# optozorax/portal

Measured on NVIDIA B200. Metric: Mpixels/s @ 3840x2160 depth-40 portal_in_portal, higher is better.
Workload: dtype f32

## Files before the change

portal_b200/csrc/device/pe_glsl.cuh:

```cuda
#pragma once

namespace pe {

#define PE_FI __forceinline__

PE_FI float radians(float d) { return d * 0.017453292519943295f; }
PE_FI float degrees(float r) { return r * 57.29577951308232f; }

PE_FI void pe_sincos_core(float x, float& s, float& c, int& q) {
    float k = ::rintf(x * 0.636619772367581343f);
    float r = ::fmaf(k, -1.5707962513f, x);
    r = ::fmaf(k, -7.5497894159e-08f, r);
    r = ::fmaf(k, -5.3903029535e-15f, r);
    float z = r * r;
    float ps = -1.9515295891e-4f;
    ps = ::fmaf(ps, z, 8.3321608736e-3f);
    ps = ::fmaf(ps, z, -1.6666654611e-1f);
    s = ::fmaf(ps * z, r, r);
    float pc = 2.443315711809948e-5f;
    pc = ::fmaf(pc, z, -1.388731625493765e-3f);
    pc = ::fmaf(pc, z, 4.166664568298827e-2f);
    c = ::fmaf(pc * z, z, ::fmaf(z, -0.5f, 1.0f));
    q = (::fabsf(k) < 1073741824.0f) ? (__float2int_rz(k) & 3) : 0;
}
// ... 116 lines not shown
}
PE_FI float log(float x) { return log2(x) * 0.69314718055994530942f; }
PE_FI float pow(float x, float y) {
    if (y == 0.0f) return 1.0f;
    if (x < 0.0f && y == ::rintf(y)) {
        const float h = y * 0.5f;
        const float r = exp2(y * log2(-x));
        return h != ::rintf(h) ? -r : r;
    }
    return exp2(y * log2(x));
}
PE_FI float sqrt(float x) { return ::sqrtf(x); }
PE_FI float inversesqrt(float x) { return 1.0f / ::sqrtf(x); }
PE_FI float abs(float x) { return ::fabsf(x); }
PE_FI int abs(int x) { return x < 0 ? -x : x; }
PE_FI float sign(float x) { return x > 0.0f ? 1.0f : (x < 0.0f ? -1.0f : 0.0f); }
PE_FI float floor(float x) { return ::floorf(x); }
PE_FI float ceil(float x) { return ::ceilf(x); }
PE_FI float fract(float x) { return x - ::floorf(x); }
PE_FI float mod(float x, float y) { return x - y * ::floorf(x / y); }
PE_FI float min(float x, float y) { return y < x ? y : x; }
PE_FI float max(float x, float y) { return x < y ? y : x; }
PE_FI int min(int x, int y) { return y < x ? y : x; }
PE_FI int max(int x, int y) { return x < y ? y : x; }
PE_FI float clamp(float x, float lo, float hi) { return min(max(x, lo), hi); }
PE_FI int clamp(int x, int lo, int hi) { return min(max(x, lo), hi); }
PE_FI float mix(float x, float y, float a) { return ::fmaf(y, a, x * (1.0f - a)); }
PE_FI float step(float edge, float x) { return x < edge ? 0.0f : 1.0f; }
PE_FI float smoothstep(float e0, float e1, float x) {
    float t = clamp((x - e0) / (e1 - e0), 0.0f, 1.0f);
    return t * t * (3.0f - 2.0f * t);
}

struct vec2;
struct vec3;
struct vec4;

struct swz2_ref {
    float &a, &b;
    PE_FI swz2_ref& operator=(const vec2& v);
    PE_FI swz2_ref& operator+=(const vec2& v);
    PE_FI swz2_ref& operator-=(const vec2& v);
    PE_FI swz2_ref& operator*=(const vec2& v);
    PE_FI swz2_ref& operator/=(const vec2& v);
    PE_FI swz2_ref& operator*=(float s) { a = a * s; b = b * s; return *this; }
    PE_FI swz2_ref& operator/=(float s) { float r = 1.0f / s; a = a * r; b = b * r; return *this; }
    PE_FI swz2_ref& operator+=(float s) { a = a + s; b = b + s; return *this; }
    PE_FI swz2_ref& operator-=(float s) { a = a - s; b = b - s; return *this; }
};
struct swz3_ref {
    float &a, &b, &c;
    PE_FI swz3_ref& operator=(const vec3& v);
    PE_FI swz3_ref& operator+=(const vec3& v);
    PE_FI swz3_ref& operator-=(const vec3& v);
    PE_FI swz3_ref& operator*=(const vec3& v);
    PE_FI swz3_ref& operator/=(const vec3& v);
    PE_FI swz3_ref& operator*=(float s) { a = a * s; b = b * s; c = c * s; return *this; }
    PE_FI swz3_ref& operator/=(float s) { float r = 1.0f / s; a = a * r; b = b * r; c = c * r; return *this; }
    PE_FI swz3_ref& operator+=(float s) { a = a + s; b = b + s; c = c + s; return *this; }
    PE_FI swz3_ref& operator-=(float s) { a = a - s; b = b - s; c = c - s; return *this; }
};
struct swz4_ref {
    float &a, &b, &c, &d;
    PE_FI swz4_ref& operator=(const vec4& v);
    PE_FI swz4_ref& operator+=(const vec4& v);
    PE_FI swz4_ref& operator-=(const vec4& v);
// ... 52 lines not shown
    PE_FI vec4(const vec3& v, float d) : x(v.x), y(v.y), z(v.z), w(d) {}
    PE_FI vec4(float a_, const vec3& v) : x(a_), y(v.x), z(v.y), w(v.z) {}
    PE_FI vec4(const vec2& u, const vec2& v) : x(u.x), y(u.y), z(v.x), w(v.y) {}
    PE_FI vec4(const vec2& u, float c, float d) : x(u.x), y(u.y), z(c), w(d) {}
    PE_FI float& operator[](int i) { return i == 0 ? x : (i == 1 ? y : (i == 2 ? z : w)); }
    PE_FI float operator[](int i) const { return i == 0 ? x : (i == 1 ? y : (i == 2 ? z : w)); }
    PE_SWZ_VEC4
};
#ifndef PE_SWZ_DEFS
#define PE_SWZ_DEFS
#endif
PE_SWZ_DEFS
#define PE_SWZ_ASSIGN(R, V, OPEQ, BODY) PE_FI R& R::operator OPEQ(const V& v) { BODY return *this; }
PE_SWZ_ASSIGN(swz2_ref, vec2, =, a = v.x; b = v.y;)
PE_SWZ_ASSIGN(swz2_ref, vec2, +=, a = a + v.x; b = b + v.y;)
PE_SWZ_ASSIGN(swz2_ref, vec2, -=, a = a - v.x; b = b - v.y;)
PE_SWZ_ASSIGN(swz2_ref, vec2, *=, a = a * v.x; b = b * v.y;)
PE_SWZ_ASSIGN(swz2_ref, vec2, /=, a = a / v.x; b = b / v.y;)
PE_SWZ_ASSIGN(swz3_ref, vec3, =, a = v.x; b = v.y; c = v.z;)
PE_SWZ_ASSIGN(swz3_ref, vec3, +=, a = a + v.x; b = b + v.y; c = c + v.z;)
PE_SWZ_ASSIGN(swz3_ref, vec3, -=, a = a - v.x; b = b - v.y; c = c - v.z;)
PE_SWZ_ASSIGN(swz3_ref, vec3, *=, a = a * v.x; b = b * v.y; c = c * v.z;)
PE_SWZ_ASSIGN(swz3_ref, vec3, /=, a = a / v.x; b = b / v.y; c = c / v.z;)
PE_SWZ_ASSIGN(swz4_ref, vec4, =, a = v.x; b = v.y; c = v.z; d = v.w;)
PE_SWZ_ASSIGN(swz4_ref, vec4, +=, a = a + v.x; b = b + v.y; c = c + v.z; d = d + v.w;)
PE_SWZ_ASSIGN(swz4_ref, vec4, -=, a = a - v.x; b = b - v.y; c = c - v.z; d = d - v.w;)
PE_SWZ_ASSIGN(swz4_ref, vec4, *=, a = a * v.x; b = b * v.y; c = c * v.z; d = d * v.w;)
PE_SWZ_ASSIGN(swz4_ref, vec4, /=, a = a / v.x; b = b / v.y; c = c / v.z; d = d / v.w;)
#undef PE_SWZ_ASSIGN
PE_FI vec2::vec2(const vec3& v) : x(v.x), y(v.y) {}
PE_FI vec2::vec2(const vec4& v) : x(v.x), y(v.y) {}
PE_FI vec3::vec3(const vec4& v) : x(v.x), y(v.y), z(v.z) {}

#define PE_V2(EX, EY) vec2(EX, EY)
#define PE_V3(EX, EY, EZ) vec3(EX, EY, EZ)
#define PE_V4(EX, EY, EZ, EW) vec4(EX, EY, EZ, EW)
#define PE_BINOPS(OP)                                                                                              \
    PE_FI vec2 operator OP(const vec2& a, const vec2& b) { return PE_V2(a.x OP b.x, a.y OP b.y); }                 \
    PE_FI vec2 operator OP(const vec2& a, float s) { return PE_V2(a.x OP s, a.y OP s); }                           \
    PE_FI vec2 operator OP(float s, const vec2& a) { return PE_V2(s OP a.x, s OP a.y); }                           \
    PE_FI vec3 operator OP(const vec3& a, const vec3& b) { return PE_V3(a.x OP b.x, a.y OP b.y, a.z OP b.z); }     \
    PE_FI vec3 operator OP(const vec3& a, float s) { return PE_V3(a.x OP s, a.y OP s, a.z OP s); }                 \
    PE_FI vec3 operator OP(float s, const vec3& a) { return PE_V3(s OP a.x, s OP a.y, s OP a.z); }                 \
    PE_FI vec4 operator OP(const vec4& a, const vec4& b) {                                                         \
        return PE_V4(a.x OP b.x, a.y OP b.y, a.z OP b.z, a.w OP b.w);                                              \
    }                                                                                                              \
    PE_FI vec4 operator OP(const vec4& a, float s) { return PE_V4(a.x OP s, a.y OP s, a.z OP s, a.w OP s); }       \
    PE_FI vec4 operator OP(float s, const vec4& a) { return PE_V4(s OP a.x, s OP a.y, s OP a.z, s OP a.w); }
PE_BINOPS(+)
PE_BINOPS(-)
PE_BINOPS(*)
#undef PE_BINOPS
PE_FI vec2 operator/(const vec2& a, const vec2& b) { return vec2(a.x / b.x, a.y / b.y); }
PE_FI vec3 operator/(const vec3& a, const vec3& b) { return vec3(a.x / b.x, a.y / b.y, a.z / b.z); }
PE_FI vec4 operator/(const vec4& a, const vec4& b) { return vec4(a.x / b.x, a.y / b.y, a.z / b.z, a.w / b.w); }
PE_FI vec2 operator/(float s, const vec2& a) { return vec2(s / a.x, s / a.y); }
PE_FI vec3 operator/(float s, const vec3& a) { return vec3(s / a.x, s / a.y, s / a.z); }
PE_FI vec4 operator/(float s, const vec4& a) { return vec4(s / a.x, s / a.y, s / a.z, s / a.w); }
PE_FI vec2 operator/(const vec2& a, float s) { float r = 1.0f / s; return vec2(a.x * r, a.y * r); }
PE_FI vec3 operator/(const vec3& a, float s) { float r = 1.0f / s; return vec3(a.x * r, a.y * r, a.z * r); }
PE_FI vec4 operator/(const vec4& a, float s) { float r = 1.0f / s; return vec4(a.x * r, a.y * r, a.z * r, a.w * r); }
PE_FI vec2 operator-(const vec2& a) { return vec2(-a.x, -a.y); }
PE_FI vec3 operator-(const vec3& a) { return vec3(-a.x, -a.y, -a.z); }
PE_FI vec4 operator-(const vec4& a) { return vec4(-a.x, -a.y, -a.z, -a.w); }

#define PE_COMPOUND(V)                                                      \
    PE_FI V& operator+=(V& a, const V& b) { a = a + b; return a; }          \
    PE_FI V& operator-=(V& a, const V& b) { a = a - b; return a; }          \
    PE_FI V& operator*=(V& a, const V& b) { a = a * b; return a; }          \
    PE_FI V& operator/=(V& a, const V& b) { a = a / b; return a; }          \
    PE_FI V& operator+=(V& a, float s) { a = a + s; return a; }             \
    PE_FI V& operator-=(V& a, float s) { a = a - s; return a; }             \
    PE_FI V& operator*=(V& a, float s) { a = a * s; return a; }             \
    PE_FI V& operator/=(V& a, float s) { a = a / s; return a; }
PE_COMPOUND(vec2)
PE_COMPOUND(vec3)
PE_COMPOUND(vec4)
#undef PE_COMPOUND

PE_FI bool operator==(const vec2& a, const vec2& b) { return a.x == b.x && a.y == b.y; }
PE_FI bool operator==(const vec3& a, const vec3& b) { return a.x == b.x && a.y == b.y && a.z == b.z; }
PE_FI bool operator==(const vec4& a, const vec4& b) { return a.x == b.x && a.y == b.y && a.z == b.z && a.w == b.w; }
PE_FI bool operator!=(const vec2& a, const vec2& b) { return !(a == b); }
// ... 361 lines not shown
```

portal_b200/csrc/pe_api.cpp:

```cpp
#include <cuda_runtime.h>
#include <dlfcn.h>
#include <nvrtc.h>
#include <sys/stat.h>
#include <unistd.h>

#include <cmath>
#include <cstdio>
#include <cstdlib>
#include <cstring>
#include <fstream>
#include <map>
#include <memory>
#include <mutex>
#include <string>
#include <type_traits>
#include <vector>

#include "../../include/portal_b200.h"
#include "pe_codegen.h"
#include "pe_driver.h"
#include "pe_internal.h"
#include "pe_kernels.h"

using namespace pe_host;

namespace {

struct PeLaunchHost {
    void* out;
    void* bounces;
    int32_t width, height;
    int32_t strip_rows, strip_first, strip_step, n_strips;
    int32_t out_full_frame;
    int32_t tiles_x, tiles_y;
    int32_t out_rgba8;
    void* queue;
    int32_t strip_shift;
    int32_t pad_;
};
static_assert(sizeof(PeLaunchHost) == 72, "PeLaunch layout");

struct Variant {
    std::string source;
    std::vector<char> cubin;
    CUmodule_t module = nullptr;
    CUfunction_t kernel = nullptr;
    CUfunction_t probe = nullptr;
    CUdeviceptr_t const_ptr = 0;
    size_t const_size = 0;
    int regs = 0;
    int blocks_per_sm = 1;
    CUmodule_t module2 = nullptr;
    CUfunction_t kernel2 = nullptr;
    CUdeviceptr_t const_ptr2 = 0;
};

struct Texture {
    void* dev = nullptr;
    int w = 0, h = 0;
};

std::string g_create_error;
std::mutex g_create_mutex;

uint64_t fnv1a(const std::string& s, uint64_t h) {
    for (unsigned char c : s) {
        h ^= c;
        h *= 1099511628211ull;
    }
    return h;
}

std::string lib_dir() {
    Dl_info info;
    if (dladdr((void*)&fnv1a, &info) && info.dli_fname) {
        std::string p = info.dli_fname;
        size_t s = p.rfind('/');
        return s == std::string::npos ? "." : p.substr(0, s);
    }
    return ".";
}

std::string cache_dir() {
    const char* e = std::getenv("PORTAL_B200_CACHE_DIR");
    std::string d = e && *e ? e : lib_dir() + "/_cache";
    mkdir(d.c_str(), 0755);
    return d;
// ... 184 lines not shown
            const float v = m[16 * slot + e];
            if (!std::isfinite(v)) finite = false;
            if (v == 0.0f) z |= 1u << e;
            else if (v == 1.0f) o |= 1u << e;
        }
        if (bottom_row_only) {
            const bool affine = (z & 0x0888u) == 0x0888u && (o & 0x8000u);
            z = affine ? 0x0888u : 0u;
            o = affine ? 0x8000u : 0u;
            if (!affine) finite = false;
        }
        return std::pair<unsigned, unsigned>{z, o | (finite ? 1u << 16 : 0u)};
    };
    for (int k = 0; k < c->layout.n_mat; k++) out[size_t(k)] = masks_of(k, false);
    const int cams[3] = {c->layout.camera_slot, c->layout.camera_slot + 2, c->layout.camera_slot + 3};
    for (int q = 0; q < 3; q++) out[size_t(c->layout.n_mat + q)] = masks_of(cams[q], true);
    return out;
}

std::vector<int> variant_key(pe_ctx* c, const std::vector<int>& ints, const std::vector<std::pair<unsigned, unsigned>>& masks) {
    std::vector<int> key;
    if (c->opts.specialize_ints) {
        key = ints;
        key[c->layout.int_slot["_ray_tracing_depth"]] = 0;
        key[c->layout.int_slot["_aa_start"]] = 0;
    }
    if (c->opts.specialize_matrices)
        for (auto& zo : masks) { key.push_back(int(zo.first)); key.push_back(int(zo.second)); }
    key.push_back(c->opts.with_probe ? 1 : 0);
    key.push_back(c->opts.uniforms_in_smem);
    key.push_back(c->opts.tile_w);
    key.push_back(c->opts.canon_rays ? 1 : 0);
    key.push_back(c->opts.w_aware ? 1 : 0);
    key.push_back(c->opts.block_threads);
    key.push_back(c->opts.min_blocks);
    key.push_back(c->opts.persistent ? 1 : 0);
    for (char d : c->opts.dynamic_ints) key.push_back(d);
    for (char d : c->opts.dynamic_mats) key.push_back(d);
    return key;
}

struct NvrtcApi {
    nvrtcResult (*Version)(int*, int*) = nullptr;
    nvrtcResult (*CreateProgram)(nvrtcProgram*, const char*, const char*, int, const char* const*, const char* const*) = nullptr;
    nvrtcResult (*CompileProgram)(nvrtcProgram, int, const char* const*) = nullptr;
    nvrtcResult (*GetProgramLogSize)(nvrtcProgram, size_t*) = nullptr;
    nvrtcResult (*GetProgramLog)(nvrtcProgram, char*) = nullptr;
    nvrtcResult (*GetCUBINSize)(nvrtcProgram, size_t*) = nullptr;
    nvrtcResult (*GetCUBIN)(nvrtcProgram, char*) = nullptr;
    nvrtcResult (*DestroyProgram)(nvrtcProgram*) = nullptr;
    const char* (*GetErrorString)(nvrtcResult) = nullptr;
    std::string why;
    bool ok = false;
};
const NvrtcApi& nvrtc_api() {
    static NvrtcApi api;
    static std::once_flag once;
    std::call_once(once, [] {
        void* h = nullptr;
        const char* env = std::getenv("PORTAL_B200_NVRTC");
        const char* candidates[] = {env && *env ? env : nullptr,
#ifdef PE_NVRTC_PATH
                                    PE_NVRTC_PATH,
#endif
                                    "/usr/local/cuda/lib64/libnvrtc.so.12", "libnvrtc.so.12", "libnvrtc.so"};
        for (const char* cnd : candidates) {
// ... 85 lines not shown

const int kMaxRespecialisations = 4;

bool select_variant(pe_ctx* c) {
    ensure_layout(c);
    std::vector<int> ints = current_ints(c);
    std::vector<std::pair<unsigned, unsigned>> masks = matrix_masks(c);
    if (c->adapt) {
        c->opts.dynamic_ints.resize(ints.size(), 0);
        c->opts.dynamic_mats.resize(masks.size(), 0);
        c->int_changes.resize(ints.size(), 0);
        c->mat_changes.resize(masks.size(), 0);
        if (c->last_ints.size() == ints.size())
            for (size_t k = 0; k < ints.size(); k++)
                if (ints[k] != c->last_ints[k] && ++c->int_changes[k] > kMaxRespecialisations) c->opts.dynamic_ints[k] = 1;
        if (c->last_masks.size() == masks.size())
            for (size_t k = 0; k < masks.size(); k++)
                if (masks[k] != c->last_masks[k] && ++c->mat_changes[k] > kMaxRespecialisations) c->opts.dynamic_mats[k] = 1;
        c->last_ints = ints;
        c->last_masks = masks;
    }
    for (size_t k = 0; k < ints.size() && k < c->opts.dynamic_ints.size(); k++)
        if (c->opts.dynamic_ints[k]) ints[k] = 0;
    for (size_t k = 0; k < masks.size() && k < c->opts.dynamic_mats.size(); k++)
        if (c->opts.dynamic_mats[k]) masks[k] = {0u, 0u};
    std::vector<int> key = variant_key(c, ints, masks);
    auto it = c->variants.find(key);
    if (it == c->variants.end()) {
        if (c->variants.size() >= 64) {
            for (auto v = c->variants.begin(); v != c->variants.end();) {
                if (v->second.get() == c->current) { ++v; continue; }
                if (v->second->module && c->has_gpu) { cudaDeviceSynchronize(); c->drv->cuModuleUnload(v->second->module); }
                if (v->second->module2 && c->has_gpu) c->drv->cuModuleUnload(v->second->module2);
                v = c->variants.erase(v);
            }
        }
        GenResult g = generate_program(c->scene, c->layout, c->opts, ints, masks);
        if (!g.error.empty()) {
            c->err = g.error;
            return false;
        }
        auto v = std::make_unique<Variant>();
        v->source = std::move(g.source);
        if (!compile_cubin(c, v->source, v->cubin)) return false;
        it = c->variants.emplace(key, std::move(v)).first;
    }
    Variant* v = it->second.get();
    if (c->has_gpu && !v->module) {
        const DriverApi* d = c->drv;
        CUresult_t r = d->cuModuleLoadData(&v->module, v->cubin.data());
        if (r != 0) {
            if (!compile_cubin(c, v->source, v->cubin, true)) return false;
            r = d->cuModuleLoadData(&v->module, v->cubin.data());
        }
        if (r != 0) { c->err = "cuModuleLoadData: " + driver_error(d, r); return false; }
        r = d->cuModuleGetFunction(&v->kernel, v->module, "pe_render_kernel");
        if (r != 0) { c->err = "cuModuleGetFunction(pe_render_kernel): " + driver_error(d, r); return false; }
        const char* block_symbol = c->opts.uniforms_in_smem ? "PE_C_UPLOAD" : "PE_C";
        r = d->cuModuleGetGlobal(&v->const_ptr, &v->const_size, v->module, block_symbol);
        if (r != 0) { c->err = std::string("cuModuleGetGlobal(") + block_symbol + "): " + driver_error(d, r); return false; }
        if (v->const_size != c->layout.size) { c->err = "constant block size mismatch between host and device"; return false; }
        if (c->opts.with_probe) {
            r = d->cuModuleGetFunction(&v->probe, v->module, "pe_probe_kernel");
            if (r != 0) { c->err = "cuModuleGetFunction(pe_probe_kernel): " + driver_error(d, r); return false; }
        }
        d->cuFuncGetAttribute(&v->regs, 4 , v->kernel);
// ... 56 lines not shown
        if (e != cudaSuccess) {
            g_create_error = std::string("cudaSetDevice: ") + cudaGetErrorString(e);
            return nullptr;
        }
        cudaDeviceProp prop;
        if (cudaGetDeviceProperties(&prop, device) == cudaSuccess) {
            c->sm_count = prop.multiProcessorCount;
            if (prop.major < 10) {
                g_create_error = "portal_b200 needs an sm_100a (B200) device; found sm_" + std::to_string(prop.major) +
                                 std::to_string(prop.minor);
                return nullptr;
            }
        }
        if (cudaStreamCreateWithFlags(&c->stream, cudaStreamNonBlocking) != cudaSuccess ||
            cudaMalloc(&c->queue_dev, 256) != cudaSuccess) {
            g_create_error = "cannot create stream / queue counter";
            if (c->stream) cudaStreamDestroy(c->stream);
            return nullptr;
        }
        c->has_gpu = true;
    }
    g_create_error.clear();
    return c.release();
}

void pe_destroy(pe_ctx* c) {
    if (!c) return;
    if (c->has_gpu) {
        cudaSetDevice(c->device);
        cudaDeviceSynchronize();
        for (auto& kv : c->variants) {
            if (kv.second->module) c->drv->cuModuleUnload(kv.second->module);
            if (kv.second->module2) c->drv->cuModuleUnload(kv.second->module2);
        }
        for (auto& kv : c->textures)
            if (kv.second.dev) cudaFree(kv.second.dev);
        if (c->scratch_dev) cudaFree(c->scratch_dev);
        if (c->scratch8_dev) cudaFree(c->scratch8_dev);
        for (auto& sl : c->slots) {
            if (sl.dev) cudaFree(sl.dev);
            if (sl.rendered) cudaEventDestroy(sl.rendered);
            if (sl.copied) cudaEventDestroy(sl.copied);
        }
        for (auto& kv : c->user_scratch)
            if (kv.second.dev) cudaFree(kv.second.dev);
        if (c->ustage) cudaFreeHost(c->ustage);
        for (auto& e : c->ustage_done) if (e) cudaEventDestroy(e);
        if (c->copy_stream) cudaStreamDestroy(c->copy_stream);
        if (c->queue_dev) cudaFree(c->queue_dev);
        if (c->stream) cudaStreamDestroy(c->stream);
    }
    delete c;
}

const char* pe_last_error(pe_ctx* c) { return c ? c->err.c_str() : g_create_error.c_str(); }

int pe_scene_begin(pe_ctx* c) {
    if (!c) return 1;
    if (c->has_gpu) {
        cudaSetDevice(c->device);
        cudaDeviceSynchronize();
        for (auto& kv : c->variants) {
            if (kv.second->module) c->drv->cuModuleUnload(kv.second->module);
            if (kv.second->module2) c->drv->cuModuleUnload(kv.second->module2);
        }
    }
    c->variants.clear();
    c->current = nullptr;
    c->scene = SceneDesc();
    c->layout_valid = false;
    c->last_ints.clear();
    c->int_changes.clear();
    c->last_masks.clear();
    c->mat_changes.clear();
    c->opts.dynamic_ints.clear();
    c->opts.dynamic_mats.clear();
    c->cblock.clear();
    c->pending_mat.clear();
    c->pending_f.clear();
    c->pending_i.clear();
    return 0;
}

#define PE_NEED(c, p)                                  \
    if (!(c)) return 1;                                \
    if (!(p)) return (c)->fail("null argument: " #p);  \
    if ((c)->layout_valid) return (c)->fail("scene description is frozen (uniforms were already set or compiled); call pe_scene_begin")

int pe_scene_add_library(pe_ctx* c, const char* name, const char* glsl) {
    PE_NEED(c, name && glsl);
    c->scene.library.push_back({name, glsl});
    return 0;
}

int pe_scene_add_material_simple(pe_ctx* c, const char* name, const double color[3], double normal_coef, int grid,
                                 double grid_scale, double grid_coef, int grid2, int grid3) {
    PE_NEED(c, name && color);
// ... 88 lines not shown
    return 0;
}

int pe_scene_declare_texture(pe_ctx* c, const char* name) {
    PE_NEED(c, name);
    c->scene.textures.push_back(name);
    return 0;
}

int pe_scene_set_skybox(pe_ctx* c, const char* texture_name) {
    PE_NEED(c, texture_name);
    c->scene.skybox = texture_name;
    return 0;
}

int pe_set_option(pe_ctx* c, const char* key, int value) {
    if (!c || !key) return 1;
    std::string k = key;
    if (k == "persistent") c->opts.persistent = value != 0;
    else if (k == "specialize_ints") c->opts.specialize_ints = value != 0;
    else if (k == "block_threads") {
        if (value < 64 || value > 1024 || value % 64) return c->fail("block_threads must be a multiple of 64 in [64, 1024]");
        c->opts.block_threads = value;
    } else if (k == "min_blocks") c->opts.min_blocks = value < 1 ? 1 : value;
    else if (k == "lineinfo") c->lineinfo = value != 0;
    else if (k == "unroll_loops") c->opts.unroll_loops = value != 0;
    else if (k == "specialize_matrices") c->opts.specialize_matrices = value != 0;
    else if (k == "hoist_planes") c->opts.hoist_planes = value != 0;
    else if (k == "lazy_planes") c->opts.lazy_planes = value != 0;
    else if (k == "with_probe") c->opts.with_probe = value != 0;
    else if (k == "adaptive") c->adapt = value != 0;
    else if (k == "canon_rays") c->opts.canon_rays = value != 0;
    else if (k == "w_aware") c->opts.w_aware = value != 0;
    else if (k == "uniforms_in_smem") {
        if (value < 0 || value > 2) return c->fail("uniforms_in_smem must be 0 (constant bank), 1 (copy loop) or 2 (TMA bulk copy)");
        c->opts.uniforms_in_smem = value;
    } else if (k == "tile_w") {
        if (value != 8 && value != 16 && value != 32) return c->fail("tile_w must be 8, 16 or 32");
        c->opts.tile_w = value;
    }
    else return c->fail("unknown option `" + k + "`");
    if (c->has_gpu) {
        cudaSetDevice(c->device);
        cudaDeviceSynchronize();
        for (auto& kv : c->variants) {
            if (kv.second->module) c->drv->cuModuleUnload(kv.second->module);
            if (kv.second->module2) c->drv->cuModuleUnload(kv.second->module2);
        }
    }
    c->variants.clear();
    c->current = nullptr;
    return 0;
}

int pe_scene_compile(pe_ctx* c) {
    if (!c) return 1;
    if (c->opts.block_threads % 64) return c->fail("block_threads must be a multiple of 64");
    return select_variant(c) ? 0 : 1;
}

const char* pe_scene_source(pe_ctx* c) { return (c && c->current) ? c->current->source.c_str() : ""; }

int pe_scene_cubin(pe_ctx* c, const void** data, size_t* size) {
    if (!c || !data || !size) return 1;
    if (!c->current) return c->fail("no compiled program");
    *data = c->current->cubin.data();
    *size = c->current->cubin.size();
    return 0;
}

int pe_scene_uniform_block(pe_ctx* c, int width, int height, const void** data, size_t* size) {
    if (!c || !data || !size) return 1;
    if (width <= 0 || height <= 0) return c->fail("pe_scene_uniform_block: bad frame size");
    ensure_layout(c);
    *fslot(c, c->layout.float_slot["_resolution_x"]) = float(width);
    *fslot(c, c->layout.float_slot["_resolution_y"]) = float(height);
    if (!select_variant(c)) return 1;
    update_derived(c);
    *data = c->cblock.data();
    *size = c->cblock.size();
// ... 74 lines not shown
    return 0;
}

size_t pe_target_pixels(const pe_target* t) {
    if (!t) return 0;
    if (t->full_frame_layout) return size_t(t->width) * size_t(t->height);
    return size_t(t->n_strips) * size_t(t->strip_rows) * size_t(t->width);
}

static bool upload_uniform_block(pe_ctx* c, CUdeviceptr_t dst, CUstream_t s) {
    const size_t n = c->cblock.size();
    const size_t stride = (n + 255) & ~size_t(255);
    if (!c->ustage || c->ustage_stride < stride) {
        if (c->ustage) { cudaDeviceSynchronize(); cudaFreeHost(c->ustage); c->ustage = nullptr; }
        if (!cuda_ok(c, cudaHostAlloc(reinterpret_cast<void**>(&c->ustage), stride * pe_ctx::kStage, cudaHostAllocDefault), "cudaHostAlloc(uniform staging)")) return false;
        c->ustage_stride = stride;
        for (int k = 0; k < pe_ctx::kStage; k++) {
            c->ustage_used[k] = false;
            if (!c->ustage_done[k] && !cuda_ok(c, cudaEventCreateWithFlags(&c->ustage_done[k], cudaEventDisableTiming), "event")) return false;
        }
    }
    const int k = c->ustage_next;
    c->ustage_next = (k + 1) % pe_ctx::kStage;
    if (c->ustage_used[k] && !cuda_ok(c, cudaEventSynchronize(c->ustage_done[k]), "uniform staging")) return false;
    uint8_t* src = c->ustage + size_t(k) * c->ustage_stride;
    std::memcpy(src, c->cblock.data(), n);
    CUresult_t r = c->drv->cuMemcpyHtoDAsync(dst, src, n, s);
    if (r != 0) { c->err = "uniform block upload: " + driver_error(c->drv, r); return false; }
    if (!cuda_ok(c, cudaEventRecord(c->ustage_done[k], (cudaStream_t)s), "event record")) return false;
    c->ustage_used[k] = true;
    return true;
}

static int render_impl(pe_ctx* c, const pe_target* t, void* out_device, void* bounces_device, void* stream, bool rgba8, int instance = 0) {
    if (!c) return 1;
    if (!out_device) return c->fail("pe_render: out_device is null");
    if (!check_target(c, t) || !bind_device(c)) return 1;
    if (t->n_strips == 0) return 0;
    ensure_layout(c);
    *fslot(c, c->layout.float_slot["_resolution_x"]) = float(t->width);
    *fslot(c, c->layout.float_slot["_resolution_y"]) = float(t->height);
    if (!select_variant(c)) return 1;
    update_derived(c);
    Variant* v = c->current;
    const DriverApi* d = c->drv;
    CUstream_t s = stream ? (CUstream_t)stream : (CUstream_t)c->stream;

    CUfunction_t kernel = v->kernel;
    CUdeviceptr_t const_ptr = v->const_ptr;
    CUresult_t r = 0;
    if (instance == 1) {
        if (!v->module2) {
            size_t sz = 0;
            r = d->cuModuleLoadData(&v->module2, v->cubin.data());
            if (r == 0) r = d->cuModuleGetFunction(&v->kernel2, v->module2, "pe_render_kernel");
            if (r == 0) r = d->cuModuleGetGlobal(&v->const_ptr2, &sz, v->module2, c->opts.uniforms_in_smem ? "PE_C_UPLOAD" : "PE_C");
            if (r != 0) return c->fail("second program instance: " + driver_error(d, r));
        }
        kernel = v->kernel2;
        const_ptr = v->const_ptr2;
    }
    if (!upload_uniform_block(c, const_ptr, s)) return 1;

    PeLaunchHost L;
    std::memset(&L, 0, sizeof L);
    L.out = out_device;
    L.bounces = bounces_device;
    L.width = t->width;
    L.height = t->height;
    L.strip_rows = t->strip_rows;
    L.strip_first = t->strip_first;
    L.strip_step = t->strip_step;
    L.n_strips = t->n_strips;
    L.out_full_frame = t->full_frame_layout ? 1 : 0;
    const int local_rows = t->n_strips * t->strip_rows;
    L.tiles_x = (t->width + 7) / 8;
    L.tiles_y = (local_rows + 3) / 4;
    L.out_rgba8 = rgba8 ? 1 : 0;
    L.queue = c->queue_dev;
    L.strip_shift = -1;
    if ((t->strip_rows & (t->strip_rows - 1)) == 0)
        for (int sh = 0; sh < 31; sh++)
            if ((1 << sh) == t->strip_rows) L.strip_shift = sh;
    void* args[] = {&L};
    unsigned gx, gy;
    if (c->opts.persistent) {
        r = d->cuMemsetD32Async((CUdeviceptr_t)c->queue_dev, 0, 1, s);
        if (r != 0) return c->fail("queue reset: " + driver_error(d, r));
        gx = unsigned(c->sm_count * v->blocks_per_sm);
        gy = 1;
    } else {
        const int tile_w = c->opts.tile_w, block_w = tile_w < 16 ? 16 : tile_w;
        const int rows_per_block = (c->opts.block_threads / 32) / (block_w / tile_w) * (32 / tile_w);
        gx = unsigned((t->width + block_w - 1) / block_w);
        gy = unsigned((local_rows + rows_per_block - 1) / rows_per_block);
    }
    r = d->cuLaunchKernel(kernel, gx, gy, 1, unsigned(c->opts.block_threads), 1, 1, 0, s, args, nullptr);
    if (r != 0) return c->fail("cuLaunchKernel(pe_render_kernel): " + driver_error(d, r));
    c->launches++;
    return 0;
}

}
int pe_internal_render_impl(pe_ctx* c, const pe_target* t, void* out_device, void* stream, int rgba8, int instance) {
    return render_impl(c, t, out_device, nullptr, stream, rgba8 != 0, instance);
}
extern "C" {

int pe_render(pe_ctx* c, const pe_target* t, void* out_device, void* bounces_device, void* stream) {
    return render_impl(c, t, out_device, bounces_device, stream, false);
}

int pe_render_rgba8(pe_ctx* c, const pe_target* t, void* out_device_rgba8, void* stream) {
    return render_impl(c, t, out_device_rgba8, nullptr, stream, true);
}

static bool ensure_scratch(pe_ctx* c, void** p, size_t* have, size_t need);

int pe_probe_ray(pe_ctx* c, const float a[3], const float b[3], float pos_out[3], int32_t* have_result,
                 int32_t* encounter_object, int32_t* change_subspace) {
    if (!c) return 1;
    if (!a || !b || !pos_out) return c->fail("pe_probe_ray: null argument");
    if (!bind_device(c)) return 1;
    ensure_layout(c);
    auto tl = c->layout.int_slot.find("teleport_light_u");
    int saved = 0;
    if (tl != c->layout.int_slot.end()) { saved = *islot(c, tl->second); *islot(c, tl->second) = 1; }
    const bool had_probe = c->opts.with_probe, had_adapt = c->adapt;
    c->opts.with_probe = true;
    c->adapt = false;
    bool ok = select_variant(c);
    c->adapt = had_adapt;
    if (ok) update_derived(c);
    struct { float ax, ay, az, bx, by, bz; void* out; } P;
    float host[6] = {0, 0, 0, 0, 0, 0};
    if (ok) {
        if (!ensure_scratch(c, &c->scratch8_dev, &c->scratch8_bytes, 64)) ok = false;
    }
    if (ok) {
        Variant* v = c->current;
        const DriverApi* d = c->drv;
        CUstream_t s = (CUstream_t)c->stream;
        P = {a[0], a[1], a[2], b[0], b[1], b[2], c->scratch8_dev};
        void* args[] = {&P};
        CUresult_t r = upload_uniform_block(c, v->const_ptr, s) ? 0 : 999;
        if (r == 0) r = d->cuLaunchKernel(v->probe, 1, 1, 1, 32, 1, 1, 0, s, args, nullptr);
        if (r != 0) { c->err = "pe_probe_kernel: " + driver_error(d, r); ok = false; }
        else {
            c->launches++;
            ok = cuda_ok(c, cudaMemcpyAsync(host, c->scratch8_dev, sizeof host, cudaMemcpyDeviceToHost, c->stream), "probe readback") &&
                 cuda_ok(c, cudaStreamSynchronize(c->stream), "pe_probe_ray");
        }
    }
    c->opts.with_probe = had_probe;
    if (tl != c->layout.int_slot.end()) *islot(c, tl->second) = saved;
    if (!ok) return 1;
    for (int k = 0; k < 3; k++) pos_out[k] = host[k];
    if (have_result) *have_result = host[3] != 0.0f;
    if (encounter_object) *encounter_object = host[4] != 0.0f;
    if (change_subspace) *change_subspace = host[5] != 0.0f;
    return 0;
}

static bool ensure_scratch(pe_ctx* c, void** p, size_t* have, size_t need) {
    if (*have >= need) return true;
    if (*p) cudaFree(*p);
    *p = nullptr;
    *have = 0;
    if (!cuda_ok(c, cudaMalloc(p, need), "cudaMalloc(staging)")) return false;
    *have = need;
    return true;
}

int pe_render_host(pe_ctx* c, const pe_target* t, float* out_host) {
    if (!c) return 1;
    if (!out_host) return c->fail("pe_render_host: out_host is null");
    if (!check_target(c, t) || !bind_device(c)) return 1;
    size_t bytes = pe_target_pixels(t) * 16;
// ... 328 lines not shown
```

portal_b200/csrc/pe_codegen.cpp:

```cpp
#include "pe_codegen.h"

#include <algorithm>
#include <cctype>
#include <cmath>
#include <cstdio>
#include <cstring>
#include <sstream>
#include <stdexcept>

#include "../../include/portal_b200.h"

namespace pe_host {

const char* const kRendererFloats[] = {"_camera_scale", "_tan_half_view", "_view_angle", "_t_start", "_t_end",
                                       "_offset_after_material", "_depth_map_min", "_depth_map_max",
                                       "_resolution_x", "_resolution_y", "_left_eye_scale", "_right_eye_scale",
                                       "_panini_param", "_anaglyph_p", "_anaglyph_q"};
const int kNumRendererFloats = int(sizeof(kRendererFloats) / sizeof(kRendererFloats[0]));
const char* const kRendererInts[] = {"_ray_tracing_depth", "_aa_start", "_aa_count", "_camera_in_subspace",
                                     "_darken_by_distance", "_angle_color_disable", "_grid_disable",
                                     "_black_border_disable", "_draw_depth_map", "_left_eye_in_subspace",
                                     "_right_eye_in_subspace", "_use_panini_projection", "_use_360_camera",
                                     "_use_180_camera", "_draw_side_by_side", "_draw_anaglyph", "_anaglyph_mode"};
const int kNumRendererInts = int(sizeof(kRendererInts) / sizeof(kRendererInts[0]));
// ... 462 lines not shown
        if (o.matrix_a != o.matrix_b && !need_mat(o.matrix_b + "_to_" + o.matrix_a, "_mat_teleport")) break;
        body.line("    } else if (i.material == teleport_" + std::to_string(pos) + "_1_M) {");
        body.line("        return material_teleport(hit, r, " + ab + ");");
        body.line("    } else if (i.material == teleport_" + std::to_string(pos) + "_2_M) {");
        body.line("        return material_teleport(hit, r, " + ba + ");");
    }
    body.line("    }");
    body.line("    return material_final(vec3(0.0f));");
    body.line("}");

    body.line("PE_FI SceneIntersectionWithMaterial scene_intersect_material_process(const Ray& r) {");
    body.line("    SceneIntersectionWithMaterial result = SceneIntersectionWithMaterial{scene_intersection_none, material_empty()};");
    if (!scene.intersection_materials.empty())
        body.line("    SceneIntersectionWithMaterial hit = result;");
    for (size_t pos = 0; pos < scene.intersection_materials.size(); pos++) {
        body.line("    hit = intersect_material_" + std::to_string(pos) + "(r);");
        body.line("    if (nearer(result.scene.hit, hit.scene.hit)) { result = hit; }");
    }
    body.line("    (void)r; return result;");
    body.line("}");

    if (!body.err.empty() && R.error.empty()) R.error = body.err;
    if (!R.error.empty()) return R;

    std::ostringstream hd;
    hd << "// GENERATED by portal_b200 (pe_codegen.cpp) -- sm_100a program of one scene.\n";
    hd << "#define PE_PERSISTENT " << (opts.persistent ? 1 : 0) << "\n";
    hd << "#define PE_BLOCK_THREADS " << opts.block_threads << "\n";
    hd << "#define PE_MIN_BLOCKS " << opts.min_blocks << "\n";
    hd << "#define PE_WITH_PROBE " << (opts.with_probe ? 1 : 0) << "\n";
    hd << "#define PE_TILE_W " << opts.tile_w << "\n";
    hd << "#define PE_CANON_RAYS " << (opts.canon_rays ? 1 : 0) << "\n";
    hd << "#define PE_W_AWARE " << ((opts.w_aware && opts.canon_rays) ? 1 : 0) << "\n";
    std::string swz_err;
    hd << "#define PE_SWZ_VEC2" << swizzle_macro(body.swz, 2) << lvalue_swizzle_macro(body.swz_w, 2, swz_err) << "\n";
    hd << "#define PE_SWZ_VEC3" << swizzle_macro(body.swz, 3) << lvalue_swizzle_macro(body.swz_w, 3, swz_err) << "\n";
    hd << "#define PE_SWZ_VEC4" << swizzle_macro(body.swz, 4) << lvalue_swizzle_macro(body.swz_w, 4, swz_err) << "\n";
    hd << "#define PE_SWZ_DEFS" << swizzle_macro(body.swz, 0) << "\n";
    if (!swz_err.empty()) { R.error = swz_err; return R; }
    hd << "#define PE_HAS_SKYBOX " << (scene.skybox.empty() ? 0 : 1) << "\n";
    {
        std::string user;
        for (const auto& lib : scene.library) user += lib.code + "\n";
        for (const char* fn : {"transpose", "inverse", "determinant"}) {
            bool defined = false;
            for (const char* ty : {"mat2", "mat3", "mat4", "float"}) {
                size_t pos = 0;
                const std::string needle = std::string(ty);
                while ((pos = user.find(needle, pos)) != std::string::npos) {
                    size_t k = pos + needle.size();
                    size_t k0 = k;
                    while (k < user.size() && std::isspace((unsigned char)user[k])) k++;
                    if (k > k0 && user.compare(k, std::strlen(fn), fn) == 0) {
                        size_t e = k + std::strlen(fn);
                        while (e < user.size() && std::isspace((unsigned char)user[e])) e++;
                        if (e < user.size() && user[e] == '(' && (pos == 0 || !is_ident_char(user[pos - 1]))) defined = true;
                    }
                    pos = k0;
                }
            }
            if (defined) hd << "#define PE_NO_BUILTIN_" << fn << "\n";
        }
    }
    hd << kSrcGlsl << "\n";
    hd << "namespace pe {\n";
    hd << "// Constant uniform block: scene matrices + camera, floats, ints, texture descriptors.\n";
// ... 95 lines not shown
```

portal_b200/csrc/pe_codegen.h:

```cpp
#pragma once
#include <cstdint>
#include <map>
#include <set>
#include <string>
#include <vector>

namespace pe_host {

enum class ObjClass { Flat, Complex, DebugMatrix };
enum class MatType { Simple, Reflect, Refract, Complex };

struct Material {
    std::string name;
    MatType type = MatType::Simple;
    double color[3] = {0, 0, 0};
    double normal_coef = 0, grid_scale = 0, grid_coef = 0, refractive_index = 0;
    bool grid = false, grid2 = false, grid3 = false;
    std::string code;
};

struct Object {
    std::string name;
    ObjClass cls = ObjClass::Flat;
    bool portal = false;
// ... 26 lines not shown
extern const char* const kRendererInts[];
extern const int kNumRendererInts;

struct PlaneRec {
    int mat_slot = 0;
    int pass_sign = 1;
    int cmp_sign = 1;
};

struct ConstLayout {
    int n_mat = 0, n_float = 0, n_int = 0, n_tex = 0;
    std::vector<std::string> mats, floats, ints;
    std::map<std::string, int> mat_slot, float_slot, int_slot, tex_slot;
    size_t off_mat = 0, off_float = 0, off_int = 0, off_tex = 0, size = 0;
    std::vector<PlaneRec> planes;
    int plane_f0 = 0, plane_i0 = 0;
    int camera_slot = 0;
};
ConstLayout make_layout(const SceneDesc& scene);

struct GenOptions {
    bool persistent = false;
    bool specialize_ints = true;
    int block_threads = 512;
    int min_blocks = 2;
    bool specialize_matrices = true;
    bool hoist_planes = true;
    bool lazy_planes = true;
    bool with_probe = false;
    int uniforms_in_smem = 0;
    int tile_w = 8;
    bool canon_rays = true;
    bool w_aware = true;
    bool unroll_loops = true;
    std::vector<char> dynamic_ints, dynamic_mats;
};

struct GenResult {
    std::string source;
    std::string error;
};

GenResult generate_program(const SceneDesc& scene, const ConstLayout& layout, const GenOptions& opts,
                           const std::vector<int>& int_values,
                           const std::vector<std::pair<unsigned, unsigned>>& matrix_masks);

std::string glsl_to_cuda(const std::string& glsl, std::set<std::string>& swizzles, bool keep_loops_rolled = false,
                         std::set<std::string>* lvalue_swizzles = nullptr);

extern const char* const kSrcGlsl;
extern const char* const kSrcLibrary;
extern const char* const kSrcKernel;

}
```

Baseline: 16850.

## Add optional packed f32x2 vector add/sub and skip redundant uniform uploads

Routes vec2/3/4 addition and subtraction through a pe_f2 helper. Behind a new pack_f32x2 option, which is off by default, that helper can use the paired __fadd2_rn instruction. Separately, each variant now keeps a copy of the uniform block resident on the device per instance and skips re-uploading it when nothing has changed. A second-instance render can also reuse instance 0's constant buffer, with an event to order any later upload. The goal is to cut per-frame host-to-device copies and, optionally, the FP32 instruction count, at the cost of added event bookkeeping and a risk of ordering hazards.

```diff
diff --git a/portal_b200/csrc/device/pe_glsl.cuh b/portal_b200/csrc/device/pe_glsl.cuh
--- a/portal_b200/csrc/device/pe_glsl.cuh
+++ b/portal_b200/csrc/device/pe_glsl.cuh
@@ -172,6 +172,21 @@
     return t * t * (3.0f - 2.0f * t);
 }
 
+#ifndef PE_PACK_F32X2
+#define PE_PACK_F32X2 0
+#endif
+struct pe_f2 { float x, y; };
+#if PE_PACK_F32X2 && defined(__CUDA_ARCH__)
+PE_FI float2 pe_to2(pe_f2 a) { return make_float2(a.x, a.y); }
+PE_FI pe_f2 pe_from2(float2 a) { return pe_f2{a.x, a.y}; }
+PE_FI pe_f2 pe_add2(pe_f2 a, pe_f2 b) { return pe_from2(__fadd2_rn(pe_to2(a), pe_to2(b))); }
+PE_FI pe_f2 pe_sub2(pe_f2 a, pe_f2 b) { return pe_from2(__fadd2_rn(pe_to2(a), make_float2(-b.x, -b.y))); }
+#else
+PE_FI pe_f2 pe_add2(pe_f2 a, pe_f2 b) { return pe_f2{a.x + b.x, a.y + b.y}; }
+PE_FI pe_f2 pe_sub2(pe_f2 a, pe_f2 b) { return pe_f2{a.x - b.x, a.y - b.y}; }
+#endif
+PE_FI pe_f2 pe_bc2(float s) { return pe_f2{s, s}; }
+
 struct vec2;
 struct vec3;
 struct vec4;
@@ -290,6 +305,26 @@
 PE_FI vec2::vec2(const vec4& v) : x(v.x), y(v.y) {}
 PE_FI vec3::vec3(const vec4& v) : x(v.x), y(v.y), z(v.z) {}
 
+PE_FI pe_f2 pe_xy(const vec2& v) { return pe_f2{v.x, v.y}; }
+PE_FI pe_f2 pe_xy(const vec3& v) { return pe_f2{v.x, v.y}; }
+PE_FI pe_f2 pe_xy(const vec4& v) { return pe_f2{v.x, v.y}; }
+PE_FI pe_f2 pe_zw(const vec4& v) { return pe_f2{v.z, v.w}; }
+PE_FI vec2 pe_v2(pe_f2 xy) { return vec2(xy.x, xy.y); }
+PE_FI vec3 pe_v3(pe_f2 xy, float z) { return vec3(xy.x, xy.y, z); }
+PE_FI vec4 pe_v4(pe_f2 xy, pe_f2 zw) { return vec4(xy.x, xy.y, zw.x, zw.y); }
+#define PE_BINOPS2(OP, F2)                                                                                                \
+    PE_FI vec2 operator OP(const vec2& a, const vec2& b) { return pe_v2(F2(pe_xy(a), pe_xy(b))); }                        \
+    PE_FI vec2 operator OP(const vec2& a, float s) { return pe_v2(F2(pe_xy(a), pe_bc2(s))); }                             \
+    PE_FI vec2 operator OP(float s, const vec2& a) { return pe_v2(F2(pe_bc2(s), pe_xy(a))); }                             \
+    PE_FI vec3 operator OP(const vec3& a, const vec3& b) { return pe_v3(F2(pe_xy(a), pe_xy(b)), a.z OP b.z); }            \
+    PE_FI vec3 operator OP(const vec3& a, float s) { return pe_v3(F2(pe_xy(a), pe_bc2(s)), a.z OP s); }                   \
+    PE_FI vec3 operator OP(float s, const vec3& a) { return pe_v3(F2(pe_bc2(s), pe_xy(a)), s OP a.z); }                   \
+    PE_FI vec4 operator OP(const vec4& a, const vec4& b) { return pe_v4(F2(pe_xy(a), pe_xy(b)), F2(pe_zw(a), pe_zw(b))); } \
+    PE_FI vec4 operator OP(const vec4& a, float s) { return pe_v4(F2(pe_xy(a), pe_bc2(s)), F2(pe_zw(a), pe_bc2(s))); }     \
+    PE_FI vec4 operator OP(float s, const vec4& a) { return pe_v4(F2(pe_bc2(s), pe_xy(a)), F2(pe_bc2(s), pe_zw(a))); }
+PE_BINOPS2(+, pe_add2)
+PE_BINOPS2(-, pe_sub2)
+#undef PE_BINOPS2
 #define PE_V2(EX, EY) vec2(EX, EY)
 #define PE_V3(EX, EY, EZ) vec3(EX, EY, EZ)
 #define PE_V4(EX, EY, EZ, EW) vec4(EX, EY, EZ, EW)
@@ -305,8 +340,6 @@
     }                                                                                                              \
     PE_FI vec4 operator OP(const vec4& a, float s) { return PE_V4(a.x OP s, a.y OP s, a.z OP s, a.w OP s); }       \
     PE_FI vec4 operator OP(float s, const vec4& a) { return PE_V4(s OP a.x, s OP a.y, s OP a.z, s OP a.w); }
-PE_BINOPS(+)
-PE_BINOPS(-)
 PE_BINOPS(*)
 #undef PE_BINOPS
 PE_FI vec2 operator/(const vec2& a, const vec2& b) { return vec2(a.x / b.x, a.y / b.y); }
diff --git a/portal_b200/csrc/pe_api.cpp b/portal_b200/csrc/pe_api.cpp
--- a/portal_b200/csrc/pe_api.cpp
+++ b/portal_b200/csrc/pe_api.cpp
@@ -53,6 +53,9 @@
     CUmodule_t module2 = nullptr;
     CUfunction_t kernel2 = nullptr;
     CUdeviceptr_t const_ptr2 = 0;
+    std::vector<uint8_t> resident[2];
+    cudaEvent_t borrowed = nullptr;
+    bool borrow_pending = false;
 };
 
 struct Texture {
@@ -303,6 +306,7 @@
     key.push_back(c->opts.tile_w);
     key.push_back(c->opts.canon_rays ? 1 : 0);
     key.push_back(c->opts.w_aware ? 1 : 0);
+    key.push_back(c->opts.pack_f32x2 ? 1 : 0);
     key.push_back(c->opts.block_threads);
     key.push_back(c->opts.min_blocks);
     key.push_back(c->opts.persistent ? 1 : 0);
@@ -454,6 +458,7 @@
                 if (v->second.get() == c->current) { ++v; continue; }
                 if (v->second->module && c->has_gpu) { cudaDeviceSynchronize(); c->drv->cuModuleUnload(v->second->module); }
                 if (v->second->module2 && c->has_gpu) c->drv->cuModuleUnload(v->second->module2);
+                if (v->second->borrowed && c->has_gpu) cudaEventDestroy(v->second->borrowed);
                 v = c->variants.erase(v);
             }
         }
@@ -576,6 +581,7 @@
         for (auto& kv : c->variants) {
             if (kv.second->module) c->drv->cuModuleUnload(kv.second->module);
             if (kv.second->module2) c->drv->cuModuleUnload(kv.second->module2);
+            if (kv.second->borrowed) cudaEventDestroy(kv.second->borrowed);
         }
         for (auto& kv : c->textures)
             if (kv.second.dev) cudaFree(kv.second.dev);
@@ -607,6 +613,7 @@
         for (auto& kv : c->variants) {
             if (kv.second->module) c->drv->cuModuleUnload(kv.second->module);
             if (kv.second->module2) c->drv->cuModuleUnload(kv.second->module2);
+            if (kv.second->borrowed) cudaEventDestroy(kv.second->borrowed);
         }
     }
     c->variants.clear();
@@ -761,6 +768,7 @@
     else if (k == "adaptive") c->adapt = value != 0;
     else if (k == "canon_rays") c->opts.canon_rays = value != 0;
     else if (k == "w_aware") c->opts.w_aware = value != 0;
+    else if (k == "pack_f32x2") c->opts.pack_f32x2 = value != 0;
     else if (k == "uniforms_in_smem") {
         if (value < 0 || value > 2) return c->fail("uniforms_in_smem must be 0 (constant bank), 1 (copy loop) or 2 (TMA bulk copy)");
         c->opts.uniforms_in_smem = value;
@@ -775,6 +783,7 @@
         for (auto& kv : c->variants) {
             if (kv.second->module) c->drv->cuModuleUnload(kv.second->module);
             if (kv.second->module2) c->drv->cuModuleUnload(kv.second->module2);
+            if (kv.second->borrowed) cudaEventDestroy(kv.second->borrowed);
         }
     }
     c->variants.clear();
@@ -915,6 +924,18 @@
     return true;
 }
 
+static bool ensure_uniform_block(pe_ctx* c, Variant* v, int inst, CUstream_t s) {
+    std::vector<uint8_t>& res = v->resident[inst];
+    if (res == c->cblock) return true;
+    if (inst == 0 && v->borrow_pending) {
+        if (!cuda_ok(c, cudaStreamWaitEvent((cudaStream_t)s, v->borrowed, 0), "uniform block ordering")) return false;
+        v->borrow_pending = false;
+    }
+    if (!upload_uniform_block(c, inst == 0 ? v->const_ptr : v->const_ptr2, s)) { res.clear(); return false; }
+    res = c->cblock;
+    return true;
+}
+
 static int render_impl(pe_ctx* c, const pe_target* t, void* out_device, void* bounces_device, void* stream, bool rgba8, int instance = 0) {
     if (!c) return 1;
     if (!out_device) return c->fail("pe_render: out_device is null");
@@ -930,8 +951,12 @@
     CUstream_t s = stream ? (CUstream_t)stream : (CUstream_t)c->stream;
 
     CUfunction_t kernel = v->kernel;
-    CUdeviceptr_t const_ptr = v->const_ptr;
     CUresult_t r = 0;
+    const bool borrow = instance == 1 && v->resident[0] == c->cblock;
+    if (borrow) {
+        if (!v->borrowed && !cuda_ok(c, cudaEventCreateWithFlags(&v->borrowed, cudaEventDisableTiming), "event")) return 1;
+        instance = 0;
+    }
     if (instance == 1) {
         if (!v->module2) {
             size_t sz = 0;
@@ -941,9 +966,8 @@
             if (r != 0) return c->fail("second program instance: " + driver_error(d, r));
         }
         kernel = v->kernel2;
-        const_ptr = v->const_ptr2;
-    }
-    if (!upload_uniform_block(c, const_ptr, s)) return 1;
+    }
+    if (!ensure_uniform_block(c, v, instance, s)) return 1;
 
     PeLaunchHost L;
     std::memset(&L, 0, sizeof L);
@@ -980,6 +1004,10 @@
     }
     r = d->cuLaunchKernel(kernel, gx, gy, 1, unsigned(c->opts.block_threads), 1, 1, 0, s, args, nullptr);
     if (r != 0) return c->fail("cuLaunchKernel(pe_render_kernel): " + driver_error(d, r));
+    if (borrow) {
+        if (!cuda_ok(c, cudaEventRecord(v->borrowed, (cudaStream_t)s), "event record")) return 1;
+        v->borrow_pending = true;
+    }
     c->launches++;
     return 0;
 }
@@ -1026,7 +1054,7 @@
         CUstream_t s = (CUstream_t)c->stream;
         P = {a[0], a[1], a[2], b[0], b[1], b[2], c->scratch8_dev};
         void* args[] = {&P};
-        CUresult_t r = upload_uniform_block(c, v->const_ptr, s) ? 0 : 999;
+        CUresult_t r = ensure_uniform_block(c, v, 0, s) ? 0 : 999;
         if (r == 0) r = d->cuLaunchKernel(v->probe, 1, 1, 1, 32, 1, 1, 0, s, args, nullptr);
         if (r != 0) { c->err = "pe_probe_kernel: " + driver_error(d, r); ok = false; }
         else {
diff --git a/portal_b200/csrc/pe_codegen.cpp b/portal_b200/csrc/pe_codegen.cpp
--- a/portal_b200/csrc/pe_codegen.cpp
+++ b/portal_b200/csrc/pe_codegen.cpp
@@ -518,6 +518,7 @@
     hd << "#define PE_TILE_W " << opts.tile_w << "\n";
     hd << "#define PE_CANON_RAYS " << (opts.canon_rays ? 1 : 0) << "\n";
     hd << "#define PE_W_AWARE " << ((opts.w_aware && opts.canon_rays) ? 1 : 0) << "\n";
+    hd << "#define PE_PACK_F32X2 " << (opts.pack_f32x2 ? 1 : 0) << "\n";
     std::string swz_err;
     hd << "#define PE_SWZ_VEC2" << swizzle_macro(body.swz, 2) << lvalue_swizzle_macro(body.swz_w, 2, swz_err) << "\n";
     hd << "#define PE_SWZ_VEC3" << swizzle_macro(body.swz, 3) << lvalue_swizzle_macro(body.swz_w, 3, swz_err) << "\n";
diff --git a/portal_b200/csrc/pe_codegen.h b/portal_b200/csrc/pe_codegen.h
--- a/portal_b200/csrc/pe_codegen.h
+++ b/portal_b200/csrc/pe_codegen.h
@@ -82,6 +82,7 @@
     int tile_w = 8;
     bool canon_rays = true;
     bool w_aware = true;
+    bool pack_f32x2 = false;
     bool unroll_loops = true;
     std::vector<char> dynamic_ints, dynamic_mats;
 };
```

New measurement: 16900, median of 6. Within noise of the previous version (+0.3%).
